# jianfenglihg/Unsupervised_depth_OpticalFlow_egomotion

Hardware: AMD Instinct MI355X
Metric: frame-pairs/sec (832x256, geom mode) (higher is better)
Workload: dtype f32; 1 GPU; train_step: mode=geom, 832x256, batch=4/GPU, num_scales=3, fwd+bwd+Adam; global_batch=4, parallelism=dp1, hw_queues=4, stream_priorities=auto

## Files before the change

### include/dfe_hip.h

```cpp
#ifndef DFE_HIP_H
#define DFE_HIP_H

#ifdef __cplusplus
extern "C" {
#endif

#define DFE_OK 0
#define DFE_ERR_NULL (-1)
#define DFE_ERR_DIMS (-2)
#define DFE_ERR_LAUNCH (-3)
#define DFE_ERR_UNSUPPORTED (-4)
#define DFE_ERR_WORKSPACE (-5)

#define DFE_MAX_SCALES 8
#define DFE_ABI_VERSION 4

int dfe_abi_version(void);
const char* dfe_error_string(int code);

int dfe_camera_floats(void);
int dfe_prepare_cameras(const float* pose, const float* K, float* cams, int B, int ndir, int nscale,
                        const float* downscale_host, void* stream);

int dfe_pose_vec2mat_fwd(const float* vec, float* T34, float* E, int n, void* stream);
// ... 121 lines not shown
int dfe_planeconv_dgrad(const float* gy, const float* weight, float* gx, float* ws, int B, int Ci, int Co, int H, int W,
                        void* stream);
int dfe_planeconv_wgrad(const float* gy, const float* x, float* gweight, float* ws, int B, int Ci, int Co, int H, int W,
                        void* stream);

long dfe_wino_weight_floats(int Ci, int Co);
long dfe_wino_scratch_floats(int B, int Ci, int Co, int H, int W, int P);
int dfe_wino_conv3x3(const float* x, const float* weight, float* y, long y_batch_stride, float* wbuf, long wbuf_floats, int B, int Ci,
                     int Co, int H, int W, int P, int transposed_weight, void* stream);
long dfe_wino_wgrad_floats(int B, int Ci, int Co, int H, int W, int P);
int dfe_wino_wgrad_tune(int tile, int blocks1, int blocks2, int chunk);
int dfe_wino_wgrad3x3(const float* x, long x_batch_stride, const float* gy, long gy_batch_stride, float* gweight, float* ws, int B,
                      int Ci, int Co, int H, int W, int P, void* stream);
int dfe_sconv_tune(int blocks, int rows);
long dfe_sconv_wgrad_floats(int B, int Ci, int Co, int H, int W, int K, int stride, int P);
int dfe_sconv_wgrad(const float* x, long x_batch_stride, const float* gy, long gy_batch_stride, float* gweight, float* ws, int B,
                    int Ci, int Co, int H, int W, int K, int stride, int P, void* stream);
long dfe_sconv_fwd_floats(int B, int Ci, int Co, int H, int W, int K);
int dfe_sconv_fwd(const float* x, long x_batch_stride, const float* weight, const float* bias, float slope, float* y,
                  long y_batch_stride, float* ws, int B, int Ci, int Co, int H, int W, int K, void* stream);
long dfe_sconv_dgrad_floats(int B, int Ci, int Co, int H, int W, int K);
int dfe_sconv_dgrad(const float* gy, long gy_batch_stride, const float* weight, float* gx, long gx_batch_stride, float* ws, int B,
                    int Ci, int Co, int H, int W, int K, void* stream);
int dfe_conv1x1s2_supported(int B, int Ci, int Co, int H, int W);
int dfe_conv1x1s2_fwd(const float* x, long x_batch_stride, const float* weight, float* y, long y_batch_stride, int B, int Ci, int Co,
                      int H, int W, void* stream);
long dfe_conv1x1s2_wgrad_floats(int B, int Ci, int Co, int H, int W);
int dfe_conv1x1s2_wgrad(const float* x, long x_batch_stride, const float* gy, long gy_batch_stride, float* gweight, float* ws, int B,
                        int Ci, int Co, int H, int W, void* stream);
int dfe_wino_conv3x3_dilated(const float* x, const float* weight, float* y, long y_batch_stride, float* wbuf, int B, int Ci, int Co,
                             int H, int W, int dilation, int transposed_weight, void* stream);
long dfe_wino_transform_blocks(int Ci, int Co);
int dfe_wino_transform_weights_multi(const long* table, const int* blockmap, int n_blocks, void* stream);
int dfe_wino_conv3x3_u(const float* x, const float* U, float* y, long y_batch_stride, float* part, long part_floats, int B, int Ci,
                       int Co, int H, int W, int P, int dilation, void* stream);
int dfe_wino_conv3x3_u_act(const float* x, const float* U, const float* bias, float slope, float* y, long y_batch_stride, float* y2,
                           long y2_batch_stride, float* part, long part_floats, int B, int Ci, int Co, int H, int W, int P,
                           int dilation, void* stream);

int dfe_conv1x1_small_supported(int B, int Ci, int Co, int H, int W);
int dfe_conv1x1_small_fwd(const float* x, const float* weight, const float* bias, float slope, float* y, int B, int Ci, int Co,
                          int H, int W, void* stream);
int dfe_conv1x1_small_bwd(const float* gy, const float* x, const float* weight, float* gx, float* gweight, int B, int Ci, int Co,
                          int H, int W, void* stream);

long dfe_bn_partials_floats(int G, int Bg, int C, int H, int W);
int dfe_bn_fwd(const float* x, const float* residual, const float* weight, const float* bias, float* running_mean,
               float* running_var, float* y, float* save_mean, float* save_invstd, float* partials, int G, int Bg, int C,
               int H, int W, float eps, float momentum, int relu, void* stream);
int dfe_bn_bwd(const float* x, const float* y, const float* gy, const float* weight, const float* save_mean,
               const float* save_invstd, float* gx, float* gres, float* gweight, float* gbias, float* partials,
               float* scratch_means, int G, int Bg, int C, int H, int W, int relu, void* stream);

int dfe_bn_fold(const float* weight, const float* bias, const float* running_mean, const float* running_var, float eps,
                float* scale, float* shift, int C, void* stream);
int dfe_bn_eval_fwd(const float* x, const float* residual, const float* scale, const float* shift, float* y, int B, int C, int H,
                    int W, int relu, void* stream);

long dfe_bias_act_partials_floats(int B, int C, int H, int W);
int dfe_bias_act_fwd(float* z, const float* bias, int B, int C, int H, int W, float slope, void* stream);
int dfe_bias_act_bwd(const float* y, const float* gy, long gy_batch_stride, float* gz, float* gbias, float* partials,
                     int B, int C, int H, int W, float slope, void* stream);

int dfe_bias_act_fwd2(const float* z, const float* bias, float* dst1, long dst1_batch_stride, float* dst2,
                      long dst2_batch_stride, int B, int C, int H, int W, float slope, void* stream);
int dfe_bias_act_bwd2(const float* y, long y_batch_stride, const float* g1, long g1_batch_stride, const float* g2,
                      long g2_batch_stride, float* gz, float* gbias, float* partials, int B, int C, int H, int W,
                      float slope, void* stream);
int dfe_bias_grad_final_multi(const float* const* partials, float* const* gbias, const int* C, int n, int B, int H, int W,
                              void* stream);

#define DFE_LOSS_DEPTH_PIXEL 0
#define DFE_LOSS_DEPTH_SMOOTH 1
#define DFE_LOSS_FLOW_PIXEL 2
#define DFE_LOSS_FLOW_SSIM 3
#define DFE_LOSS_FLOW_SMOOTH 4
#define DFE_LOSS_FLOW_CONSIS 5
#define DFE_LOSS_DEPTH_FLOW_CONSIS 6
#define DFE_LOSS_EPIPOLAR 7
#define DFE_LOSS_DEPTH_SSIM 8
#define DFE_LOSS_DEPTH_CONSIS 9
#define DFE_NUM_LOSSES 10
#define DFE_DEPTH_TERM_SSIM 1
#define DFE_DEPTH_TERM_CONSIS 2

#define DFE_MASK_VALID_BWD 0x01
#define DFE_MASK_VALID_FWD 0x02
#define DFE_MASK_OCC_BWD 0x04
#define DFE_MASK_OCC_FWD 0x08
#define DFE_MASK_DYNA_BWD 0x10
#define DFE_MASK_DYNA_FWD 0x20
#define DFE_MASK_TEX_BWD 0x40
#define DFE_MASK_TEX_FWD 0x80

typedef struct dfe_geom_args {
  int B, H, W;
  int num_scales;
  int align_corners;
  int mode;
  float alpha, beta;
  const float* img[3];
  const float* disp[3][DFE_MAX_SCALES];
  const float* flow[2][DFE_MAX_SCALES];
  const float* pose;
  const float* K;
  const float* K_inv;
// ... 33 lines not shown
```

### unsupervised_depth_opticalflow_egomotion_amd/csrc/dfe_internal.h

```cpp
#pragma once
#include <hip/hip_runtime.h>
#include <cstdint>
#include <cstdlib>
#include "../../include/dfe_hip.h"

#define DFE_LAUNCH_CHECK() do { if (hipGetLastError() != hipSuccess) return DFE_ERR_LAUNCH; } while (0)

namespace dfe {
struct ScaleList { float v[DFE_MAX_SCALES]; };
struct IntList { int v[DFE_MAX_SCALES]; };

inline int launch_status() { return hipGetLastError() == hipSuccess ? DFE_OK : DFE_ERR_LAUNCH; }
inline int env_int(const char* name, int dflt) { const char* e = getenv(name); return e ? atoi(e) : dflt; }
inline bool aligned8(const void* p) { return (reinterpret_cast<uintptr_t>(p) & 7) == 0; }
inline bool aligned16(const void* p) { return (reinterpret_cast<uintptr_t>(p) & 15) == 0; }
inline bool sample_ok(long bs, long per) { return bs >= per && per < (1L << 30); }
template <auto Kern, class... Args>
inline void launch_dyn_lds(unsigned grid, size_t lds_bytes, int attr_bytes, hipStream_t st, Args... args) {
  static bool attr_set = false;
  if (!attr_set) { (void)hipFuncSetAttribute(reinterpret_cast<const void*>(Kern), hipFuncAttributeMaxDynamicSharedMemorySize, attr_bytes); attr_set = true; }
  Kern<<<grid, 256, lds_bytes, st>>>(args...);
}

int launch_corr_fwd(const float* f1, const float* f2, float* out, long obs, float* tail, const float* flow, int B, int C, int H, int W,
                    hipStream_t st);
int launch_corr_bwd(const float* f1, const float* f2, const float* gout, long gbs, const float* add1, long abs1, float* g1,
                    float* g2, unsigned* amax2, int B, int C, int H, int W, hipStream_t st);

int launch_bias_final(const float* part, float* gbias, int B, int C, int n, hipStream_t st);
}
```

### unsupervised_depth_opticalflow_egomotion_amd/csrc/ops_bn.hip

```cpp
#include "dfe_internal.h"
#include "dfe_device.h"
#include "dfe_chunk.h"
#include <hip/hip_runtime.h>

namespace dfe {

constexpr int BN_BLOCK = CHUNK_BLOCK;
constexpr int BN_PER_THREAD = CHUNK_PER_THREAD;
constexpr int BN_CHUNK = CHUNK_ELEMS;

__device__ __forceinline__ float block_allsum(float v, float* smem) {
  v = dpp_add<0xB1>(v); v = dpp_add<0x4E>(v); v = dpp_add<0x141>(v); v = dpp_add<0x140>(v);
  const int lane = threadIdx.x & 63, wave = threadIdx.x >> 6;
  if ((lane & 15) == 0) smem[wave * 4 + (lane >> 4)] = v;
  __syncthreads();
  float s = 0.0f;
#pragma unroll
  for (int k = 0; k < 4 * (BN_BLOCK / 64); ++k) s += smem[k];
  __syncthreads();
  return s;
}

template <bool VEC>
__global__ void __launch_bounds__(BN_BLOCK) k_bn_stats(const float* __restrict__ x, float* __restrict__ part, int HW) {
// ... 364 lines not shown
    if (VEC) {
#pragma unroll
      for (int k = 0; k < BNE_PER_LANE / 4; ++k) {
        const int e = base + (k * 64 + lane) * 4;
        float4 q = make_float4(0.f, 0.f, 0.f, 0.f), p = q;
        if (e < HW) {
          q = *reinterpret_cast<const float4*>(x + off + e);
          if (RES) p = *reinterpret_cast<const float4*>(res + off + e);
        }
        v[4 * k] = q.x; v[4 * k + 1] = q.y; v[4 * k + 2] = q.z; v[4 * k + 3] = q.w;
        r[4 * k] = p.x; r[4 * k + 1] = p.y; r[4 * k + 2] = p.z; r[4 * k + 3] = p.w;
      }
    } else {
#pragma unroll
      for (int k = 0; k < BNE_PER_LANE; ++k) {
        const int e = base + k * 64 + lane;
        v[k] = e < HW ? x[off + e] : 0.0f;
        r[k] = (RES && e < HW) ? res[off + e] : 0.0f;
      }
    }
#pragma unroll
    for (int k = 0; k < BNE_PER_LANE; ++k) {
      float o = v[k] * s;
      o = o + t;
      if (RES) o = o + r[k];
      v[k] = (relu && o <= 0.0f) ? 0.0f : o;
    }
    if (VEC) {
#pragma unroll
      for (int k = 0; k < BNE_PER_LANE / 4; ++k) {
        const int e = base + (k * 64 + lane) * 4;
        if (e < HW) *reinterpret_cast<float4*>(y + off + e) = make_float4(v[4 * k], v[4 * k + 1], v[4 * k + 2], v[4 * k + 3]);
      }
    } else {
#pragma unroll
      for (int k = 0; k < BNE_PER_LANE; ++k) {
        const int e = base + k * 64 + lane;
        if (e < HW) y[off + e] = v[k];
      }
    }
  }
}

}

using namespace dfe;

static inline int bn_nchunk(long hw) { return static_cast<int>((hw + BN_CHUNK - 1) / BN_CHUNK); }

static int bn_dims(int G, int Bg, int C, int H, int W) {
  const long hw = static_cast<long>(H) * W;
  if (G <= 0 || Bg <= 0 || C <= 0 || H <= 0 || W <= 0 || hw >= (1L << 31) || C > 65535 || static_cast<long>(G) * Bg > 65535) return DFE_ERR_DIMS;
  if (static_cast<long>(Bg) * hw < 2) return DFE_ERR_DIMS;
  return DFE_OK;
}

extern "C" long dfe_bn_partials_floats(int G, int Bg, int C, int H, int W) {
  if (bn_dims(G, Bg, C, H, W) != DFE_OK) return 0;
  return static_cast<long>(G) * Bg * C * bn_nchunk(static_cast<long>(H) * W) * 3;
}

extern "C" int dfe_bn_fwd(const float* x, const float* residual, const float* weight, const float* bias, float* running_mean,
                          float* running_var, float* y, float* save_mean, float* save_invstd, float* partials, int G, int Bg,
                          int C, int H, int W, float eps, float momentum, int relu, void* stream) {
  if (!x || !y || !save_mean || !save_invstd || !partials) return DFE_ERR_NULL;
  int rc = bn_dims(G, Bg, C, H, W);
  if (rc != DFE_OK) return rc;
  const int hw = H * W, nchunk = bn_nchunk(hw);
  const dim3 grid(nchunk, C, G * Bg);
  hipStream_t st = static_cast<hipStream_t>(stream);
  const bool vec = hw % 4 == 0 && aligned16(x) && aligned16(y) && (!residual || aligned16(residual));
  if (vec && hw <= BNS_MAXHW && Bg <= BNS_MAXB) {
#define DFE_BNS_FWD(GB, T) k_bn_fwd_small<GB, T><<<C, T, 0, st>>>(x, residual, weight, bias, running_mean, running_var, y, \
                                                                save_mean, save_invstd, G, Bg, C, hw, eps, momentum, relu)
    if (G == 3) { if (hw <= 256) DFE_BNS_FWD(3, 64); else if (hw <= 1024) DFE_BNS_FWD(3, 256); else DFE_BNS_FWD(3, 1024); }
    else { if (hw <= 256) DFE_BNS_FWD(1, 64); else if (hw <= 1024) DFE_BNS_FWD(1, 256); else DFE_BNS_FWD(1, 1024); }
#undef DFE_BNS_FWD
    DFE_LAUNCH_CHECK();
    return DFE_OK;
  }
  if (vec) k_bn_stats<true><<<grid, BN_BLOCK, 0, st>>>(x, partials, hw);
  else k_bn_stats<false><<<grid, BN_BLOCK, 0, st>>>(x, partials, hw);
  DFE_LAUNCH_CHECK();
  k_bn_finalize<<<C, 64, 0, st>>>(partials, save_mean, save_invstd, running_mean, running_var, G, Bg, C, nchunk, eps, momentum);
  DFE_LAUNCH_CHECK();
  if (vec) k_bn_apply<true><<<grid, BN_BLOCK, 0, st>>>(x, residual, weight, bias, save_mean, save_invstd, y, Bg, C, hw, relu);
  else k_bn_apply<false><<<grid, BN_BLOCK, 0, st>>>(x, residual, weight, bias, save_mean, save_invstd, y, Bg, C, hw, relu);
  DFE_LAUNCH_CHECK();
  return DFE_OK;
}

extern "C" int dfe_bn_bwd(const float* x, const float* y, const float* gy, const float* weight, const float* save_mean,
                          const float* save_invstd, float* gx, float* gres, float* gweight, float* gbias, float* partials,
                          float* scratch_means, int G, int Bg, int C, int H, int W, int relu, void* stream) {
  if (!x || !gy || !save_mean || !save_invstd || !gx || !partials || !scratch_means || (relu && !y)) return DFE_ERR_NULL;
  int rc = bn_dims(G, Bg, C, H, W);
  if (rc != DFE_OK) return rc;
  const int hw = H * W, nchunk = bn_nchunk(hw);
  const dim3 grid(nchunk, C, G * Bg);
  hipStream_t st = static_cast<hipStream_t>(stream);
  float* gmean = scratch_means;
  float* gxmean = scratch_means + static_cast<long>(G) * C;
  const bool vec = hw % 4 == 0 && aligned16(x) && aligned16(gy) && aligned16(gx) && (!relu || aligned16(y)) && (!gres || aligned16(gres));
  if (vec && hw <= BNS_MAXHW && Bg <= BNS_MAXB) {
#define DFE_BNS_BWD(GB, T) k_bn_bwd_small<GB, T><<<C, T, 0, st>>>(x, y, gy, weight, save_mean, save_invstd, gx, gres, gweight, \
                                                                gbias, G, Bg, C, hw, relu)
    if (G == 3) { if (hw <= 256) DFE_BNS_BWD(3, 64); else if (hw <= 1024) DFE_BNS_BWD(3, 256); else DFE_BNS_BWD(3, 1024); }
    else { if (hw <= 256) DFE_BNS_BWD(1, 64); else if (hw <= 1024) DFE_BNS_BWD(1, 256); else DFE_BNS_BWD(1, 1024); }
#undef DFE_BNS_BWD
    DFE_LAUNCH_CHECK();
    return DFE_OK;
  }
  if (vec) k_bn_bwd_reduce<true><<<grid, BN_BLOCK, 0, st>>>(x, y, gy, save_mean, save_invstd, partials, Bg, C, hw, relu);
  else k_bn_bwd_reduce<false><<<grid, BN_BLOCK, 0, st>>>(x, y, gy, save_mean, save_invstd, partials, Bg, C, hw, relu);
  DFE_LAUNCH_CHECK();
  k_bn_bwd_finalize<<<C, 64, 0, st>>>(partials, gmean, gxmean, gweight, gbias, G, Bg, C, nchunk, hw);
  DFE_LAUNCH_CHECK();
  if (vec) k_bn_bwd_apply<true><<<grid, BN_BLOCK, 0, st>>>(x, y, gy, weight, save_mean, save_invstd, gmean, gxmean, gx, gres, Bg, C, hw, relu);
  else k_bn_bwd_apply<false><<<grid, BN_BLOCK, 0, st>>>(x, y, gy, weight, save_mean, save_invstd, gmean, gxmean, gx, gres, Bg, C, hw, relu);
  DFE_LAUNCH_CHECK();
  return DFE_OK;
}

extern "C" int dfe_bn_fold(const float* weight, const float* bias, const float* running_mean, const float* running_var, float eps,
                           float* scale, float* shift, int C, void* stream) {
  if (!running_mean || !running_var || !scale || !shift) return DFE_ERR_NULL;
  if (C <= 0) return DFE_ERR_DIMS;
  k_bn_fold<<<(C + 63) / 64, 64, 0, static_cast<hipStream_t>(stream)>>>(weight, bias, running_mean, running_var, eps, scale, shift, C);
  DFE_LAUNCH_CHECK();
  return DFE_OK;
}

extern "C" int dfe_bn_eval_fwd(const float* x, const float* residual, const float* scale, const float* shift, float* y, int B, int C,
                               int H, int W, int relu, void* stream) {
  if (!x || !scale || !shift || !y) return DFE_ERR_NULL;
  const long hw = static_cast<long>(H) * W;
  if (B <= 0 || C <= 0 || H <= 0 || W <= 0 || hw >= (1L << 31)) return DFE_ERR_DIMS;
  const long nchunk = (hw + BNE_WAVE_ELEMS - 1) / BNE_WAVE_ELEMS, units = static_cast<long>(B) * C * nchunk;
  if (units >= (1L << 30)) return DFE_ERR_DIMS;
  const long blocks = (units + BNE_WAVES - 1) / BNE_WAVES;
  const int grid = static_cast<int>(blocks < BNE_MAX_BLOCKS ? blocks : BNE_MAX_BLOCKS);
  hipStream_t st = static_cast<hipStream_t>(stream);
  const bool vec = hw % 4 == 0 && aligned16(x) && aligned16(y) && (!residual || aligned16(residual));
#define DFE_BNE(VEC, RES) k_bn_eval<VEC, RES><<<grid, BNE_BLOCK, 0, st>>>(x, residual, scale, shift, y, C, static_cast<int>(hw), \
                                                                          static_cast<int>(nchunk), static_cast<int>(units), relu)
  if (vec) { if (residual) DFE_BNE(true, true); else DFE_BNE(true, false); }
  else { if (residual) DFE_BNE(false, true); else DFE_BNE(false, false); }
#undef DFE_BNE
  DFE_LAUNCH_CHECK();
  return DFE_OK;
}
```

### unsupervised_depth_opticalflow_egomotion_amd/csrc/ops_pool.hip

```cpp
#include "dfe_device.h"
#include "dfe_internal.h"
#include <cmath>

namespace dfe {

constexpr int PL_ROWS = 8;

struct Row3 { float v0, v1, v2; };

__device__ __forceinline__ Row3 pool_row(const float* __restrict__ plane, int r, int H, int W, int ox, bool lane_live) {
  const float ninf = -INFINITY;
  Row3 o{ninf, ninf, ninf};
  const bool rok = lane_live && r >= 0 && r < H;
  const int c1 = 2 * ox;
  if (rok) {
    const float* row = plane + static_cast<long>(r) * W;
    if (c1 + 1 < W) { const PairF p = *reinterpret_cast<const PairF*>(row + c1); o.v1 = p.a; o.v2 = p.b; }
    else o.v1 = row[c1];
  }
  const float left = wave_shr1(o.v2);
  o.v0 = left;
  if ((threadIdx.x & 63) == 0) o.v0 = (rok && c1 - 1 >= 0) ? plane[static_cast<long>(r) * W + c1 - 1] : ninf;
  if (ox == 0) o.v0 = ninf;
  return o;
}

__device__ __forceinline__ void pool_scan(const Row3& r, int base, float& best, int& bi, bool& seeded, int rr, int H, int ox, int W, int oy) {
  const int row = 2 * oy - 1 + rr;
  if (row < 0 || row >= H) return;
  const float v[3] = {r.v0, r.v1, r.v2};
#pragma unroll
  for (int cc = 0; cc < 3; ++cc) {
    const int col = 2 * ox - 1 + cc;
    if (col < 0 || col >= W) continue;
    if (!seeded) { bi = base + cc; seeded = true; }
    if (v[cc] > best || v[cc] != v[cc]) { best = v[cc]; bi = base + cc; }
  }
}

__global__ void __launch_bounds__(64) k_maxpool3x3s2_fwd(const float* __restrict__ x, float* __restrict__ y,
                                                         unsigned char* __restrict__ idx, int H, int W, int Ho, int Wo,
                                                         int strips) {
  const int strip = blockIdx.x % strips, rb = blockIdx.x / strips;
  const long pl = blockIdx.y;
  const int ox = strip * 64 + static_cast<int>(threadIdx.x);
  const bool live = ox < Wo;
  const float* plane = x + pl * H * W;
  const int oy0 = rb * PL_ROWS, oy1 = min(oy0 + PL_ROWS, Ho);
  Row3 top = pool_row(plane, 2 * oy0 - 1, H, W, ox, live);
  for (int oy = oy0; oy < oy1; ++oy) {
    const Row3 mid = pool_row(plane, 2 * oy, H, W, ox, live);
    const Row3 bot = pool_row(plane, 2 * oy + 1, H, W, ox, live);
    float best = -INFINITY;
    int bi = 0;
    bool seeded = false;
    pool_scan(top, 0, best, bi, seeded, 0, H, ox, W, oy);
    pool_scan(mid, 3, best, bi, seeded, 1, H, ox, W, oy);
    pool_scan(bot, 6, best, bi, seeded, 2, H, ox, W, oy);
    if (live) {
      const long o = (pl * Ho + oy) * Wo + ox;
      y[o] = best;
      idx[o] = static_cast<unsigned char>(bi);
    }
    top = bot;
  }
}

struct GI { float g; int k; };

__device__ __forceinline__ GI pool_gi(const float* __restrict__ gy, const unsigned char* __restrict__ idx, long plane_off,
                                      int oy, int ox, int Ho, int Wo) {
  GI r{0.0f, -1};
  if (oy >= 0 && oy < Ho && ox >= 0 && ox < Wo) {
    const long o = plane_off + static_cast<long>(oy) * Wo + ox;
    r.g = gy[o]; r.k = idx[o];
  }
  return r;
}

__global__ void __launch_bounds__(64) k_maxpool3x3s2_bwd(const float* __restrict__ gy, const unsigned char* __restrict__ idx,
                                                         float* __restrict__ gx, int H, int W, int Ho, int Wo, int strips) {
  const int strip = blockIdx.x % strips, rb = blockIdx.x / strips;
  const long pl = blockIdx.y;
  const int ox = strip * 64 + static_cast<int>(threadIdx.x);
  const int c1 = 2 * ox, c2 = 2 * ox + 1;
  if (c1 >= W) return;
  const long po = pl * Ho * Wo;
  float* plane = gx + pl * H * W;
  const int oy0 = rb * PL_ROWS, oy1 = min(oy0 + PL_ROWS, Ho);
  GI pa = pool_gi(gy, idx, po, oy0 - 1, ox, Ho, Wo), pb = pool_gi(gy, idx, po, oy0 - 1, ox + 1, Ho, Wo);
// ... 52 lines not shown
```

### unsupervised_depth_opticalflow_egomotion_amd/networks/depth_model.py

```python
import numpy as np
import torch
import torch.nn as nn
import torch.nn.functional as F

from . import resnet
from .. import convs, ops


class ResnetEncoder(nn.Module):
    def __init__(self, num_layers=18, pretrained=False):
        super().__init__()
        if num_layers not in (18, 34):
            raise ValueError("{} is not a valid number of resnet layers".format(num_layers))
        self.num_ch_enc = np.array([64, 64, 128, 256, 512])
        self.encoder = {18: resnet.resnet18, 34: resnet.resnet34}[num_layers](pretrained)

    def forward(self, image):
        e = self.encoder
        x = (image - 0.45) / 0.225
        f0 = e.bn1(e.conv1(x), relu=True)
        f1 = e.layer1(e.maxpool(f0))
        f2 = e.layer2(f1)
        f3 = e.layer3(f2)
        f4 = e.layer4(f3)
        return [f0, f1, f2, f3, f4]


class Conv3x3(nn.Module):

    def __init__(self, cin, cout):
        super().__init__()
        self.pad = nn.ReflectionPad2d(1)
        self.conv = nn.Conv2d(int(cin), int(cout), 3)

    def forward(self, x):
        return self.conv(self.pad(x))


class ConvBlock(nn.Module):

    def __init__(self, cin, cout):
        super().__init__()
        self.conv = Conv3x3(cin, cout)
        self.nonlin = nn.ELU(inplace=True)

    def forward(self, x):
        return self.nonlin(self.conv(x))


class DepthDecoder(nn.Module):
    def __init__(self, num_ch_enc, scales=range(4)):
        super().__init__()
        self.scales = list(scales)
        self.num_ch_enc = num_ch_enc
        self.num_ch_dec = np.array([16, 32, 64, 128, 256])
        self.upconvs = nn.ModuleList()
        for i in range(4, -1, -1):
            cin = num_ch_enc[-1] if i == 4 else self.num_ch_dec[i + 1]
            pair = nn.ModuleList([ConvBlock(cin, self.num_ch_dec[i])])
            cin2 = self.num_ch_dec[i] + (num_ch_enc[i - 1] if i > 0 else 0)
            pair.append(ConvBlock(cin2, self.num_ch_dec[i]))
            self.upconvs.append(pair)
        self.dispconvs = nn.ModuleList([Conv3x3(self.num_ch_dec[s], 1) for s in self.scales])
        self.sigmoid = nn.Sigmoid()

    def forward(self, feats):
        return self.forward_fused(feats) if feats[-1].is_cuda else self.forward_aten(feats)

    def forward_aten(self, feats):
        out = {}
        x = feats[-1]
        for scale in range(4, -1, -1):
            blk = self.upconvs[4 - scale]
            x = blk[0](x)
# ... 58 lines not shown
```

### unsupervised_depth_opticalflow_egomotion_amd/networks/resnet.py

```python
import torch
import torch.nn as nn
import torch.nn.functional as F

from .. import ops
from ..convs import Conv2d


class FrameBatchNorm2d(nn.BatchNorm2d):
    groups = 1
    count_deferred = False
    folded = None

    def forward(self, x, residual=None, relu=False):
        if self.folded is not None and x.is_cuda and not self.training:
            return ops.bn_eval(x, self.folded[0], self.folded[1], residual=residual, relu=relu, out=x if x.is_contiguous() else None)
        if x.is_cuda and self.training:
            if self.momentum is None or not self.track_running_stats or not self.affine:
                raise ValueError("FrameBatchNorm2d: only affine, momentum-tracked batch norm is implemented in HIP")
            if not self.count_deferred:
                self.num_batches_tracked.add_(self.groups)
            return ops.grouped_batch_norm(x, self.weight, self.bias, self.running_mean, self.running_var, self.groups,
                                          self.eps, self.momentum, residual=residual, relu=relu)
        if self.training and self.groups > 1:
            y = torch.cat([super(FrameBatchNorm2d, self).forward(c) for c in x.chunk(self.groups, 0)], 0)
        else:
            y = super().forward(x)
        if residual is not None:
            y = y + residual
        return F.relu(y) if relu else y


class StemMaxPool(nn.MaxPool2d):

    def forward(self, x):
        if x.is_cuda and (self.kernel_size, self.stride, self.padding, self.dilation, self.ceil_mode) == (3, 2, 1, 1, False) \
                and x.dim() == 4 and x.shape[0] * x.shape[1] <= 65535:
            return ops.maxpool3x3s2(x)
        return super().forward(x)


class BasicBlock(nn.Module):
    expansion = 1

    def __init__(self, inplanes, planes, stride=1, downsample=None):
        super().__init__()
        self.conv1 = Conv2d(inplanes, planes, 3, stride, 1, bias=False)
        self.bn1 = FrameBatchNorm2d(planes)
        self.relu = nn.ReLU(inplace=True)
        self.conv2 = Conv2d(planes, planes, 3, 1, 1, bias=False)
        self.bn2 = FrameBatchNorm2d(planes)
        self.downsample = downsample
        self.stride = stride

    def forward(self, x):
        idt = x if self.downsample is None else self.downsample(x)
        out = self.bn1(self.conv1(x), relu=True)
        return self.bn2(self.conv2(out), residual=idt, relu=True)


class ResNet(nn.Module):
    def __init__(self, block, layers, num_classes=1000):
        super().__init__()
        self.inplanes = 64
        self.conv1 = Conv2d(3, 64, 7, 2, 3, bias=False)
        self.bn1 = FrameBatchNorm2d(64)
        self.relu = nn.ReLU(inplace=True)
        self.maxpool = StemMaxPool(3, 2, 1)
        self.layer1 = self._make_layer(block, 64, layers[0])
        self.layer2 = self._make_layer(block, 128, layers[1], stride=2)
        self.layer3 = self._make_layer(block, 256, layers[2], stride=2)
        self.layer4 = self._make_layer(block, 512, layers[3], stride=2)
        self.avgpool = nn.AdaptiveAvgPool2d((1, 1))
        self.fc = nn.Linear(512 * block.expansion, num_classes)
        for m in self.modules():
            if isinstance(m, nn.Conv2d):
                nn.init.kaiming_normal_(m.weight, mode="fan_out", nonlinearity="relu")
            elif isinstance(m, nn.BatchNorm2d):
                nn.init.constant_(m.weight, 1)
                nn.init.constant_(m.bias, 0)

    def _make_layer(self, block, planes, blocks, stride=1):
        down = None
        if stride != 1 or self.inplanes != planes * block.expansion:
            down = nn.Sequential(Conv2d(self.inplanes, planes * block.expansion, 1, stride, bias=False),
                                 FrameBatchNorm2d(planes * block.expansion))
        layers = [block(self.inplanes, planes, stride, down)]
        self.inplanes = planes * block.expansion
        layers += [block(self.inplanes, planes) for _ in range(1, blocks)]
        return nn.Sequential(*layers)

    def forward(self, x):
        x = self.maxpool(self.bn1(self.conv1(x), relu=True))
        x = self.layer4(self.layer3(self.layer2(self.layer1(x))))
        return self.fc(self.avgpool(x).flatten(1))


def resnet18(pretrained=False, **kw):
    if pretrained:
        raise RuntimeError("no network access: pretrained ImageNet weights are unavailable")
    return ResNet(BasicBlock, [2, 2, 2, 2], **kw)


def resnet34(pretrained=False, **kw):
    if pretrained:
        raise RuntimeError("no network access: pretrained ImageNet weights are unavailable")
    return ResNet(BasicBlock, [3, 4, 6, 3], **kw)
```

### unsupervised_depth_opticalflow_egomotion_amd/ops.py

```python
from __future__ import annotations

import ctypes
import os
import threading

import torch

from . import _lib
from ._lib import DfeError, check, f32c, get_lib, ptr, stream_ptr

_ALIGN_CORNERS = False


def set_align_corners(flag: bool):
    global _ALIGN_CORNERS
    _ALIGN_CORNERS = bool(flag)


def get_align_corners() -> bool:
    return _ALIGN_CORNERS


def _ac(flag):
    return int(_ALIGN_CORNERS if flag is None else bool(flag))
# ... 1031 lines not shown
    @staticmethod
    def forward(ctx, x, residual, weight, bias, running_mean, running_var, groups, eps, momentum, relu):
        lib = get_lib()
        x = f32c(x)
        N, C, H, W = x.shape
        G = int(groups)
        if N % G:
            raise ValueError("batch %d is not divisible into %d groups" % (N, G))
        Bg = N // G
        residual = f32c(residual) if residual is not None else None
        if residual is not None and residual.shape != x.shape:
            raise ValueError("residual must have the shape of x")
        dev = x.device
        y = torch.empty_like(x)
        mean = torch.empty(G * C, device=dev)
        invstd = torch.empty(G * C, device=dev)
        npart = lib.dfe_bn_partials_floats(G, Bg, C, H, W)
        part = torch.empty(max(npart, 1), device=dev)
        check(lib.dfe_bn_fwd(ptr(x), ptr(residual), ptr(weight), ptr(bias), ptr(running_mean), ptr(running_var), ptr(y),
                             ptr(mean), ptr(invstd), ptr(part), G, Bg, C, H, W, float(eps), float(momentum), int(relu),
                             stream_ptr()), "dfe_bn_fwd")
        ctx.save_for_backward(x, y if relu else x.new_empty(0), weight if weight is not None else x.new_empty(0), mean, invstd)
        ctx.cfg = (G, Bg, C, H, W, int(relu), residual is not None, weight is not None)
        ctx.mark_non_differentiable(mean, invstd)
        return y

    @staticmethod
    def backward(ctx, gy):
        lib = get_lib()
        x, y, weight, mean, invstd = ctx.saved_tensors
        G, Bg, C, H, W, relu, has_res, has_w = ctx.cfg
        gy = f32c(gy)
        dev = x.device
        gx = torch.empty_like(x)
        gres = (torch.empty_like(x) if relu else None) if (has_res and ctx.needs_input_grad[1]) else None
        gw = torch.empty(C, device=dev) if (has_w and ctx.needs_input_grad[2]) else None
        gb = torch.empty(C, device=dev) if ctx.needs_input_grad[3] else None
        part = torch.empty(max(lib.dfe_bn_partials_floats(G, Bg, C, H, W), 1), device=dev)
        scratch = torch.empty(2 * G * C, device=dev)
        check(lib.dfe_bn_bwd(ptr(x), ptr(y) if relu else None, ptr(gy), ptr(weight) if has_w else None, ptr(mean), ptr(invstd),
                             ptr(gx), ptr(gres), ptr(gw), ptr(gb), ptr(part), ptr(scratch), G, Bg, C, H, W, relu,
                             stream_ptr()), "dfe_bn_bwd")
        if has_res and ctx.needs_input_grad[1] and not relu:
            gres = gy
        return gx, gres, gw, gb, None, None, None, None, None, None


def grouped_batch_norm(x, weight, bias, running_mean, running_var, groups=1, eps=1e-5, momentum=0.1, residual=None,
                       relu=False):
    return GroupedBatchNormFn.apply(x, residual, weight, bias, running_mean, running_var, int(groups), float(eps),
                                    float(momentum), bool(relu))


def _forward_only(what, *tensors):
    if torch.is_grad_enabled() and any(t is not None and t.requires_grad for t in tensors):
        raise DfeError("%s is forward-only (it has no backward pass): call it under torch.no_grad(), or detach its inputs" % what)


def bn_fold(bn, out=None):
    if bn.running_mean is None or bn.running_var is None:
        raise DfeError("bn_fold: the layer tracks no running statistics")
    _forward_only("bn_fold", bn.weight, bn.bias, bn.running_mean, bn.running_var)
    C = int(bn.running_mean.numel())
    scale, shift = out if out is not None else (torch.empty(C, device=bn.running_mean.device, dtype=torch.float32) for _ in range(2))
    for t in (scale, shift):
        if t.dtype != torch.float32 or t.numel() != C:
            raise DfeError("bn_fold: out must be two fp32 tensors of %d elements" % C)
    w, b = (None if t is None else f32c(t.detach()) for t in (bn.weight, bn.bias))
    check(get_lib().dfe_bn_fold(ptr(w), ptr(b), ptr(f32c(bn.running_mean)), ptr(f32c(bn.running_var)), float(bn.eps), ptr(scale),
                                ptr(shift), C, stream_ptr()), "dfe_bn_fold")
    return scale, shift


def bn_eval(x, scale, shift, residual=None, relu=False, out=None):
    _forward_only("bn_eval", x, scale, shift, residual)
    if x.dim() != 4:
        raise DfeError("bn_eval: x must be [B,C,H,W], got %s" % (tuple(x.shape),))
    x = x if out is x else f32c(x)
    B, C, H, W = x.shape
    residual = f32c(residual) if residual is not None else None
    if residual is not None and residual.shape != x.shape:
        raise DfeError("bn_eval: residual must have the shape of x")
    if any(t.dtype != torch.float32 or t.numel() != C for t in (scale, shift)):
        raise DfeError("bn_eval: scale / shift must be fp32 tensors of %d channels (ops.bn_fold's)" % C)
    y = torch.empty_like(x) if out is None else out
    if y.shape != x.shape or y.dtype != torch.float32 or x.dtype != torch.float32:
        raise DfeError("bn_eval: out must be an fp32 tensor of the shape of x")
    if residual is not None and residual.data_ptr() == y.data_ptr():
        raise DfeError("bn_eval: residual must not alias out")
    check(get_lib().dfe_bn_eval_fwd(ptr(x), ptr(residual), ptr(scale), ptr(shift), ptr(y), B, C, H, W, int(bool(relu)), stream_ptr()),
          "dfe_bn_eval_fwd")
    return y


class DispHeadFn(torch.autograd.Function):

    @staticmethod
    def forward(ctx, p, weight, bias):
        lib = get_lib()
        p, weight = f32c(p), f32c(weight)
        bias = f32c(bias) if bias is not None else None
        B, C, Hp, Wp = p.shape
        if tuple(weight.shape) != (1, C, 3, 3):
            raise ValueError("weight must be [1,%d,3,3], got %s" % (C, tuple(weight.shape)))
        H, W = Hp - 2, Wp - 2
        out = torch.empty(B, 1, H, W, device=p.device)
# ... 70 lines not shown
```

Baseline: 434.3 frame-pairs/s.

## Fuse ResNet stem BatchNorm apply, ReLU and 3x3 max-pool into one kernel pair

Adds a fused stem op that computes BN statistics, then applies the BN affine and ReLU while producing the stride-2 3x3 max-pool output and argmax positions in a single pass. The backward routes pooled gradients back through the stored argmax and the ReLU mask inside the BN backward reduce and apply kernels, so no separate maxpool backward or intermediate gradient tensor is needed. This cuts kernel launches and full-resolution memory traffic for the stem. In exchange it adds more complex index logic, extra uint8 position storage, and recomputes the pool-gradient scatter in both the reduce and the apply kernel.

```diff
diff --git a/include/dfe_hip.h b/include/dfe_hip.h
--- a/include/dfe_hip.h
+++ b/include/dfe_hip.h
@@ -197,6 +197,13 @@
                const float* save_invstd, float* gx, float* gres, float* gweight, float* gbias, float* partials,
                float* scratch_means, int G, int Bg, int C, int H, int W, int relu, void* stream);
 
+int dfe_bn_relu_pool_fwd(const float* x, const float* weight, const float* bias, float* running_mean, float* running_var,
+                         float* f0, float* pooled, unsigned char* pos, float* save_mean, float* save_invstd, float* partials,
+                         int G, int Bg, int C, int H, int W, float eps, float momentum, void* stream);
+int dfe_bn_relu_pool_bwd(const float* x, const float* weight, const float* bias, const float* save_mean, const float* save_invstd,
+                         const float* g_f0, const float* g_pooled, const unsigned char* pos, float* gx, float* gweight,
+                         float* gbias, float* partials, float* scratch_means, int G, int Bg, int C, int H, int W, void* stream);
+
 int dfe_bn_fold(const float* weight, const float* bias, const float* running_mean, const float* running_var, float eps,
                 float* scale, float* shift, int C, void* stream);
 int dfe_bn_eval_fwd(const float* x, const float* residual, const float* scale, const float* shift, float* y, int B, int C, int H,
diff --git a/unsupervised_depth_opticalflow_egomotion_amd/csrc/dfe_internal.h b/unsupervised_depth_opticalflow_egomotion_amd/csrc/dfe_internal.h
--- a/unsupervised_depth_opticalflow_egomotion_amd/csrc/dfe_internal.h
+++ b/unsupervised_depth_opticalflow_egomotion_amd/csrc/dfe_internal.h
@@ -27,5 +27,10 @@
 int launch_corr_bwd(const float* f1, const float* f2, const float* gout, long gbs, const float* add1, long abs1, float* g1,
                     float* g2, unsigned* amax2, int B, int C, int H, int W, hipStream_t st);
 
+int launch_bn_stats(const float* x, float* running_mean, float* running_var, float* save_mean, float* save_invstd, float* partials,
+                    int G, int Bg, int C, int H, int W, bool vec, float eps, float momentum, hipStream_t st);
+int launch_bn_bwd_finalize(const float* partials, float* gmean, float* gxmean, float* gweight, float* gbias, int G, int Bg, int C,
+                           int H, int W, hipStream_t st);
+
 int launch_bias_final(const float* part, float* gbias, int B, int C, int n, hipStream_t st);
 }
diff --git a/unsupervised_depth_opticalflow_egomotion_amd/csrc/dfe_pool.h b/unsupervised_depth_opticalflow_egomotion_amd/csrc/dfe_pool.h
--- /dev/null
+++ b/unsupervised_depth_opticalflow_egomotion_amd/csrc/dfe_pool.h
@@ -0,0 +1,23 @@
+#pragma once
+#include <hip/hip_runtime.h>
+
+namespace dfe {
+
+constexpr int PL_ROWS = 8;
+
+struct Row3 { float v0, v1, v2; };
+
+__device__ __forceinline__ void pool_scan(const Row3& r, int base, float& best, int& bi, bool& seeded, int rr, int H, int ox, int W, int oy) {
+  const int row = 2 * oy - 1 + rr;
+  if (row < 0 || row >= H) return;
+  const float v[3] = {r.v0, r.v1, r.v2};
+#pragma unroll
+  for (int cc = 0; cc < 3; ++cc) {
+    const int col = 2 * ox - 1 + cc;
+    if (col < 0 || col >= W) continue;
+    if (!seeded) { bi = base + cc; seeded = true; }
+    if (v[cc] > best || v[cc] != v[cc]) { best = v[cc]; bi = base + cc; }
+  }
+}
+
+}
diff --git a/unsupervised_depth_opticalflow_egomotion_amd/csrc/ops_bn.hip b/unsupervised_depth_opticalflow_egomotion_amd/csrc/ops_bn.hip
--- a/unsupervised_depth_opticalflow_egomotion_amd/csrc/ops_bn.hip
+++ b/unsupervised_depth_opticalflow_egomotion_amd/csrc/ops_bn.hip
@@ -440,6 +440,29 @@
   const long hw = static_cast<long>(H) * W;
   if (G <= 0 || Bg <= 0 || C <= 0 || H <= 0 || W <= 0 || hw >= (1L << 31) || C > 65535 || static_cast<long>(G) * Bg > 65535) return DFE_ERR_DIMS;
   if (static_cast<long>(Bg) * hw < 2) return DFE_ERR_DIMS;
+  return DFE_OK;
+}
+
+int dfe::launch_bn_stats(const float* x, float* running_mean, float* running_var, float* save_mean, float* save_invstd,
+                         float* partials, int G, int Bg, int C, int H, int W, bool vec, float eps, float momentum, hipStream_t st) {
+  const int rc = bn_dims(G, Bg, C, H, W);
+  if (rc != DFE_OK) return rc;
+  const int hw = H * W, nchunk = bn_nchunk(hw);
+  const dim3 grid(nchunk, C, G * Bg);
+  if (vec) k_bn_stats<true><<<grid, BN_BLOCK, 0, st>>>(x, partials, hw);
+  else k_bn_stats<false><<<grid, BN_BLOCK, 0, st>>>(x, partials, hw);
+  DFE_LAUNCH_CHECK();
+  k_bn_finalize<<<C, 64, 0, st>>>(partials, save_mean, save_invstd, running_mean, running_var, G, Bg, C, nchunk, eps, momentum);
+  DFE_LAUNCH_CHECK();
+  return DFE_OK;
+}
+
+int dfe::launch_bn_bwd_finalize(const float* partials, float* gmean, float* gxmean, float* gweight, float* gbias, int G, int Bg,
+                                int C, int H, int W, hipStream_t st) {
+  const int rc = bn_dims(G, Bg, C, H, W);
+  if (rc != DFE_OK) return rc;
+  k_bn_bwd_finalize<<<C, 64, 0, st>>>(partials, gmean, gxmean, gweight, gbias, G, Bg, C, bn_nchunk(static_cast<long>(H) * W), H * W);
+  DFE_LAUNCH_CHECK();
   return DFE_OK;
 }
 
@@ -467,11 +490,8 @@
     DFE_LAUNCH_CHECK();
     return DFE_OK;
   }
-  if (vec) k_bn_stats<true><<<grid, BN_BLOCK, 0, st>>>(x, partials, hw);
-  else k_bn_stats<false><<<grid, BN_BLOCK, 0, st>>>(x, partials, hw);
-  DFE_LAUNCH_CHECK();
-  k_bn_finalize<<<C, 64, 0, st>>>(partials, save_mean, save_invstd, running_mean, running_var, G, Bg, C, nchunk, eps, momentum);
-  DFE_LAUNCH_CHECK();
+  rc = launch_bn_stats(x, running_mean, running_var, save_mean, save_invstd, partials, G, Bg, C, H, W, vec, eps, momentum, st);
+  if (rc != DFE_OK) return rc;
   if (vec) k_bn_apply<true><<<grid, BN_BLOCK, 0, st>>>(x, residual, weight, bias, save_mean, save_invstd, y, Bg, C, hw, relu);
   else k_bn_apply<false><<<grid, BN_BLOCK, 0, st>>>(x, residual, weight, bias, save_mean, save_invstd, y, Bg, C, hw, relu);
   DFE_LAUNCH_CHECK();
@@ -502,8 +522,8 @@
   if (vec) k_bn_bwd_reduce<true><<<grid, BN_BLOCK, 0, st>>>(x, y, gy, save_mean, save_invstd, partials, Bg, C, hw, relu);
   else k_bn_bwd_reduce<false><<<grid, BN_BLOCK, 0, st>>>(x, y, gy, save_mean, save_invstd, partials, Bg, C, hw, relu);
   DFE_LAUNCH_CHECK();
-  k_bn_bwd_finalize<<<C, 64, 0, st>>>(partials, gmean, gxmean, gweight, gbias, G, Bg, C, nchunk, hw);
-  DFE_LAUNCH_CHECK();
+  rc = launch_bn_bwd_finalize(partials, gmean, gxmean, gweight, gbias, G, Bg, C, H, W, st);
+  if (rc != DFE_OK) return rc;
   if (vec) k_bn_bwd_apply<true><<<grid, BN_BLOCK, 0, st>>>(x, y, gy, weight, save_mean, save_invstd, gmean, gxmean, gx, gres, Bg, C, hw, relu);
   else k_bn_bwd_apply<false><<<grid, BN_BLOCK, 0, st>>>(x, y, gy, weight, save_mean, save_invstd, gmean, gxmean, gx, gres, Bg, C, hw, relu);
   DFE_LAUNCH_CHECK();
diff --git a/unsupervised_depth_opticalflow_egomotion_amd/csrc/ops_pool.hip b/unsupervised_depth_opticalflow_egomotion_amd/csrc/ops_pool.hip
--- a/unsupervised_depth_opticalflow_egomotion_amd/csrc/ops_pool.hip
+++ b/unsupervised_depth_opticalflow_egomotion_amd/csrc/ops_pool.hip
@@ -1,12 +1,9 @@
 #include "dfe_device.h"
 #include "dfe_internal.h"
+#include "dfe_pool.h"
 #include <cmath>
 
 namespace dfe {
-
-constexpr int PL_ROWS = 8;
-
-struct Row3 { float v0, v1, v2; };
 
 __device__ __forceinline__ Row3 pool_row(const float* __restrict__ plane, int r, int H, int W, int ox, bool lane_live) {
   const float ninf = -INFINITY;
@@ -23,19 +20,6 @@
   if ((threadIdx.x & 63) == 0) o.v0 = (rok && c1 - 1 >= 0) ? plane[static_cast<long>(r) * W + c1 - 1] : ninf;
   if (ox == 0) o.v0 = ninf;
   return o;
-}
-
-__device__ __forceinline__ void pool_scan(const Row3& r, int base, float& best, int& bi, bool& seeded, int rr, int H, int ox, int W, int oy) {
-  const int row = 2 * oy - 1 + rr;
-  if (row < 0 || row >= H) return;
-  const float v[3] = {r.v0, r.v1, r.v2};
-#pragma unroll
-  for (int cc = 0; cc < 3; ++cc) {
-    const int col = 2 * ox - 1 + cc;
-    if (col < 0 || col >= W) continue;
-    if (!seeded) { bi = base + cc; seeded = true; }
-    if (v[cc] > best || v[cc] != v[cc]) { best = v[cc]; bi = base + cc; }
-  }
 }
 
 __global__ void __launch_bounds__(64) k_maxpool3x3s2_fwd(const float* __restrict__ x, float* __restrict__ y,
diff --git a/unsupervised_depth_opticalflow_egomotion_amd/csrc/ops_stem.hip b/unsupervised_depth_opticalflow_egomotion_amd/csrc/ops_stem.hip
--- /dev/null
+++ b/unsupervised_depth_opticalflow_egomotion_amd/csrc/ops_stem.hip
@@ -0,0 +1,253 @@
+#include "dfe_device.h"
+#include "dfe_internal.h"
+#include "dfe_chunk.h"
+#include "dfe_pool.h"
+#include <cmath>
+
+namespace dfe {
+
+struct StemAffine { float mu, is, sc, sh; };
+
+__device__ __forceinline__ StemAffine stem_affine(const float* __restrict__ weight, const float* __restrict__ bias,
+                                                  const float* __restrict__ mean, const float* __restrict__ invstd, int plane,
+                                                  int Bg, int C) {
+  const int n = plane / C, c = plane - n * C, g = n / Bg;
+  const float is = invstd[g * C + c];
+  return StemAffine{mean[g * C + c], is, is * (weight ? weight[c] : 1.0f), bias ? bias[c] : 0.0f};
+}
+
+__device__ __forceinline__ float stem_pre(float v, const StemAffine& a) { return (v - a.mu) * a.sc + a.sh; }
+__device__ __forceinline__ float stem_act(float v, const StemAffine& a) {
+  const float o = stem_pre(v, a);
+  return o <= 0.0f ? 0.0f : o;
+}
+
+constexpr int ST_IN_ROWS = 2 * PL_ROWS + 1;
+
+__global__ void __launch_bounds__(64) k_stem_apply_pool(const float* __restrict__ x, const float* __restrict__ weight,
+                                                        const float* __restrict__ bias, const float* __restrict__ mean,
+                                                        const float* __restrict__ invstd, float* __restrict__ f0,
+                                                        float* __restrict__ y, unsigned char* __restrict__ idx, int Bg, int C,
+                                                        int H, int W, int Ho, int Wo, int strips) {
+  const int strip = blockIdx.x % strips, rb = blockIdx.x / strips;
+  const long pl = blockIdx.y;
+  const StemAffine a = stem_affine(weight, bias, mean, invstd, static_cast<int>(blockIdx.y), Bg, C);
+  const int ox = strip * 64 + static_cast<int>(threadIdx.x);
+  const bool live = ox < Wo;
+  const int c1 = 2 * ox;
+  const bool pair = c1 + 1 < W;
+  const bool first = threadIdx.x == 0;
+  const float* xp = x + pl * H * W;
+  float* fp = f0 + pl * H * W;
+  const int oy0 = rb * PL_ROWS, oy1 = min(oy0 + PL_ROWS, Ho);
+  const int r0 = 2 * oy0 - 1;
+  float xa[ST_IN_ROWS], xb[ST_IN_ROWS], xl[ST_IN_ROWS];
+#pragma unroll
+  for (int t = 0; t < ST_IN_ROWS; ++t) {
+    const int r = r0 + t;
+    xa[t] = 0.0f; xb[t] = 0.0f; xl[t] = 0.0f;
+    if (live && r >= 0 && r < H) {
+      const float* row = xp + static_cast<long>(r) * W;
+      if (pair) { const PairF p = *reinterpret_cast<const PairF*>(row + c1); xa[t] = p.a; xb[t] = p.b; }
+      else xa[t] = row[c1];
+      if (first && ox > 0) xl[t] = row[c1 - 1];
+    }
+  }
+  const float ninf = -INFINITY;
+  auto make_row = [&](int t) -> Row3 {
+    const int r = r0 + t;
+    const bool rok = live && r >= 0 && r < H;
+    Row3 o{ninf, ninf, ninf};
+    if (rok) {
+      o.v1 = stem_act(xa[t], a);
+      if (pair) o.v2 = stem_act(xb[t], a);
+      if (t > 0) {
+        float* row = fp + static_cast<long>(r) * W;
+        if (pair) *reinterpret_cast<PairF*>(row + c1) = PairF{o.v1, o.v2}; else row[c1] = o.v1;
+      }
+    }
+    o.v0 = wave_shr1(o.v2);
+    if (first) o.v0 = (rok && ox > 0) ? stem_act(xl[t], a) : ninf;
+    if (ox == 0) o.v0 = ninf;
+    return o;
+  };
+  Row3 top = make_row(0);
+#pragma unroll
+  for (int i = 0; i < PL_ROWS; ++i) {
+    const int oy = oy0 + i;
+    if (oy >= oy1) break;
+    const Row3 mid = make_row(2 * i + 1);
+    const Row3 bot = make_row(2 * i + 2);
+    float best = ninf;
+    int bi = 0;
+    bool seeded = false;
+    pool_scan(top, 0, best, bi, seeded, 0, H, ox, W, oy);
+    pool_scan(mid, 3, best, bi, seeded, 1, H, ox, W, oy);
+    pool_scan(bot, 6, best, bi, seeded, 2, H, ox, W, oy);
+    if (live) {
+      const long o = (pl * Ho + oy) * Wo + ox;
+      y[o] = best;
+      idx[o] = static_cast<unsigned char>(bi);
+    }
+    top = bot;
+  }
+}
+
+struct PoolGrad { const float* g; const unsigned char* k; int W, Ho, Wo; };
+
+__device__ __forceinline__ void stem_adj_row1(const PoolGrad& p, int oy, int wr, int c, float& s) {
+  if (oy >= p.Ho) return;
+  const long o = static_cast<long>(oy) * p.Wo + (c >> 1);
+  const int b = 3 * wr;
+  const int k0 = p.k[o];
+  const float g0 = p.g[o];
+  if ((c & 1) == 0) { if (k0 == b + 1) s += g0; return; }
+  const bool second = (c >> 1) + 1 < p.Wo;
+  const int k1 = second ? p.k[o + 1] : -1;
+  const float g1 = second ? p.g[o + 1] : 0.0f;
+  if (k0 == b + 2) s += g0;
+  if (k1 == b) s += g1;
+}
+
+__device__ __forceinline__ void stem_adj_row4(const PoolGrad& p, int oy, int wr, int c0, float (&s)[4]) {
+  if (oy >= p.Ho) return;
+  const long o = static_cast<long>(oy) * p.Wo + (c0 >> 1);
+  const int b = 3 * wr;
+  const bool third = (c0 >> 1) + 2 < p.Wo;
+  const int k0 = p.k[o], k1 = p.k[o + 1], k2 = third ? p.k[o + 2] : -1;
+  const float g0 = p.g[o], g1 = p.g[o + 1], g2 = third ? p.g[o + 2] : 0.0f;
+  if (k0 == b + 1) s[0] += g0;
+  if (k0 == b + 2) s[1] += g0;
+  if (k1 == b) s[1] += g1;
+  if (k1 == b + 1) s[2] += g1;
+  if (k1 == b + 2) s[3] += g1;
+  if (k2 == b) s[3] += g2;
+}
+
+template <bool VEC>
+__device__ __forceinline__ void stem_grad8(const float* __restrict__ xp, const float* __restrict__ gsp, const PoolGrad& p,
+                                           const StemAffine& a, int base, int HW, float (&v)[CHUNK_PER_THREAD],
+                                           float (&gm)[CHUNK_PER_THREAD]) {
+  bool ok[CHUNK_PER_THREAD];
+  float gs[CHUNK_PER_THREAD], adj[CHUNK_PER_THREAD];
+  load8<VEC>(xp, base, HW, v, ok);
+  if (gsp) load8<VEC>(gsp, base, HW, gs, ok);
+#pragma unroll
+  for (int k = 0; k < CHUNK_PER_THREAD; ++k) adj[k] = 0.0f;
+  if (p.g) {
+    if (VEC && p.W % 4 == 0) {
+#pragma unroll
+      for (int q = 0; q < CHUNK_PER_THREAD / 4; ++q) {
+        const int e = base + (q * CHUNK_BLOCK + static_cast<int>(threadIdx.x)) * 4;
+        if (e >= HW) continue;
+        const int r = e / p.W, c0 = e - r * p.W;
+        float s[4] = {0.0f, 0.0f, 0.0f, 0.0f};
+        if (r & 1) { stem_adj_row4(p, (r - 1) >> 1, 2, c0, s); stem_adj_row4(p, (r + 1) >> 1, 0, c0, s); }
+        else stem_adj_row4(p, r >> 1, 1, c0, s);
+#pragma unroll
+        for (int j = 0; j < 4; ++j) adj[4 * q + j] = s[j];
+      }
+    } else {
+#pragma unroll
+      for (int k = 0; k < CHUNK_PER_THREAD; ++k) {
+        const int e = VEC ? base + ((k >> 2) * CHUNK_BLOCK + static_cast<int>(threadIdx.x)) * 4 + (k & 3)
+                          : base + k * CHUNK_BLOCK + static_cast<int>(threadIdx.x);
+        if (e >= HW) continue;
+        const int r = e / p.W, c = e - r * p.W;
+        float s = 0.0f;
+        if (r & 1) { stem_adj_row1(p, (r - 1) >> 1, 2, c, s); stem_adj_row1(p, (r + 1) >> 1, 0, c, s); }
+        else stem_adj_row1(p, r >> 1, 1, c, s);
+        adj[k] = s;
+      }
+    }
+  }
+#pragma unroll
+  for (int k = 0; k < CHUNK_PER_THREAD; ++k) {
+    const float g = p.g ? (gsp ? gs[k] + adj[k] : adj[k]) : gs[k];
+    gm[k] = (!ok[k] || stem_pre(v[k], a) <= 0.0f) ? 0.0f : g;
+  }
+}
+
+#define DFE_STEM_BWD_PARAMS const float* __restrict__ x, const float* __restrict__ g_f0, const float* __restrict__ g_pooled, \
+    const unsigned char* __restrict__ pos, const float* __restrict__ weight, const float* __restrict__ bias,                 \
+    const float* __restrict__ mean, const float* __restrict__ invstd
+
+template <bool VEC>
+__global__ void __launch_bounds__(CHUNK_BLOCK) k_stem_bwd_reduce(DFE_STEM_BWD_PARAMS, float* __restrict__ part, int Bg, int C,
+                                                                 int H, int W, int Ho, int Wo) {
+  __shared__ float red[2 * 4 * (CHUNK_BLOCK / 64)];
+  const long pl = plane_id();
+  const StemAffine a = stem_affine(weight, bias, mean, invstd, static_cast<int>(pl), Bg, C);
+  const PoolGrad p{g_pooled ? g_pooled + pl * Ho * Wo : nullptr, pos + pl * Ho * Wo, W, Ho, Wo};
+  const int HW = H * W, base = blockIdx.x * CHUNK_ELEMS;
+  float v[CHUNK_PER_THREAD], gm[CHUNK_PER_THREAD];
+  stem_grad8<VEC>(x + pl * HW, g_f0 ? g_f0 + pl * HW : nullptr, p, a, base, HW, v, gm);
+  float acc[2] = {0.0f, 0.0f};
+#pragma unroll
+  for (int k = 0; k < CHUNK_PER_THREAD; ++k) {
+    acc[0] += gm[k];
+    acc[1] += gm[k] * ((v[k] - a.mu) * a.is);
+  }
+  block_sum<2>(acc, red, part + (pl * gridDim.x + blockIdx.x) * 2);
+}
+
+template <bool VEC>
+__global__ void __launch_bounds__(CHUNK_BLOCK) k_stem_bwd_apply(DFE_STEM_BWD_PARAMS, const float* __restrict__ gmean,
+                                                                const float* __restrict__ gxmean, float* __restrict__ gx, int Bg,
+                                                                int C, int H, int W, int Ho, int Wo) {
+  const long pl = plane_id();
+  const StemAffine a = stem_affine(weight, bias, mean, invstd, static_cast<int>(pl), Bg, C);
+  const int n = static_cast<int>(pl) / C, c = static_cast<int>(pl) - n * C, g = n / Bg;
+  const float ws = (weight ? weight[c] : 1.0f) * a.is, m0 = gmean[g * C + c], m1 = gxmean[g * C + c];
+  const PoolGrad p{g_pooled ? g_pooled + pl * Ho * Wo : nullptr, pos + pl * Ho * Wo, W, Ho, Wo};
+  const int HW = H * W, base = blockIdx.x * CHUNK_ELEMS;
+  float v[CHUNK_PER_THREAD], gm[CHUNK_PER_THREAD];
+  stem_grad8<VEC>(x + pl * HW, g_f0 ? g_f0 + pl * HW : nullptr, p, a, base, HW, v, gm);
+#pragma unroll
+  for (int k = 0; k < CHUNK_PER_THREAD; ++k) v[k] = ws * ((gm[k] - m0) - ((v[k] - a.mu) * a.is) * m1);
+  store8<VEC>(gx + pl * HW, base, HW, v);
+}
+#undef DFE_STEM_BWD_PARAMS
+
+}
+
+using namespace dfe;
+
+extern "C" int dfe_bn_relu_pool_fwd(const float* x, const float* weight, const float* bias, float* running_mean, float* running_var,
+                                    float* f0, float* pooled, unsigned char* pos, float* save_mean, float* save_invstd,
+                                    float* partials, int G, int Bg, int C, int H, int W, float eps, float momentum, void* stream) {
+  if (!x || !f0 || !pooled || !pos || !save_mean || !save_invstd || !partials) return DFE_ERR_NULL;
+  if (G <= 0 || Bg <= 0 || C <= 0 || static_cast<long>(G) * Bg * C > 65535) return DFE_ERR_DIMS;
+  hipStream_t st = static_cast<hipStream_t>(stream);
+  const bool vec = (static_cast<long>(H) * W) % 4 == 0 && aligned16(x) && aligned16(f0);
+  const int rc = launch_bn_stats(x, running_mean, running_var, save_mean, save_invstd, partials, G, Bg, C, H, W, vec, eps, momentum, st);
+  if (rc != DFE_OK) return rc;
+  const int Ho = dfe_maxpool3x3s2_out(H), Wo = dfe_maxpool3x3s2_out(W);
+  const int strips = (Wo + 63) / 64, rbs = (Ho + PL_ROWS - 1) / PL_ROWS;
+  k_stem_apply_pool<<<dim3(strips * rbs, G * Bg * C), 64, 0, st>>>(x, weight, bias, save_mean, save_invstd, f0, pooled, pos, Bg, C,
+                                                                  H, W, Ho, Wo, strips);
+  return launch_status();
+}
+
+extern "C" int dfe_bn_relu_pool_bwd(const float* x, const float* weight, const float* bias, const float* save_mean,
+                                    const float* save_invstd, const float* g_f0, const float* g_pooled, const unsigned char* pos,
+                                    float* gx, float* gweight, float* gbias, float* partials, float* scratch_means, int G, int Bg,
+                                    int C, int H, int W, void* stream) {
+  if (!x || !save_mean || !save_invstd || !pos || !gx || !partials || !scratch_means || (!g_f0 && !g_pooled)) return DFE_ERR_NULL;
+  if (dfe_bn_partials_floats(G, Bg, C, H, W) == 0) return DFE_ERR_DIMS;
+  hipStream_t st = static_cast<hipStream_t>(stream);
+  const int hw = H * W, nchunk = (hw + CHUNK_ELEMS - 1) / CHUNK_ELEMS;
+  const int Ho = dfe_maxpool3x3s2_out(H), Wo = dfe_maxpool3x3s2_out(W);
+  const dim3 grid(nchunk, C, G * Bg);
+  float* gmean = scratch_means;
+  float* gxmean = scratch_means + static_cast<long>(G) * C;
+  const bool vec = hw % 4 == 0 && aligned16(x) && aligned16(gx) && (!g_f0 || aligned16(g_f0));
+  if (vec) k_stem_bwd_reduce<true><<<grid, CHUNK_BLOCK, 0, st>>>(x, g_f0, g_pooled, pos, weight, bias, save_mean, save_invstd, partials, Bg, C, H, W, Ho, Wo);
+  else k_stem_bwd_reduce<false><<<grid, CHUNK_BLOCK, 0, st>>>(x, g_f0, g_pooled, pos, weight, bias, save_mean, save_invstd, partials, Bg, C, H, W, Ho, Wo);
+  DFE_LAUNCH_CHECK();
+  const int rc = launch_bn_bwd_finalize(partials, gmean, gxmean, gweight, gbias, G, Bg, C, H, W, st);
+  if (rc != DFE_OK) return rc;
+  if (vec) k_stem_bwd_apply<true><<<grid, CHUNK_BLOCK, 0, st>>>(x, g_f0, g_pooled, pos, weight, bias, save_mean, save_invstd, gmean, gxmean, gx, Bg, C, H, W, Ho, Wo);
+  else k_stem_bwd_apply<false><<<grid, CHUNK_BLOCK, 0, st>>>(x, g_f0, g_pooled, pos, weight, bias, save_mean, save_invstd, gmean, gxmean, gx, Bg, C, H, W, Ho, Wo);
+  return launch_status();
+}
diff --git a/unsupervised_depth_opticalflow_egomotion_amd/networks/depth_model.py b/unsupervised_depth_opticalflow_egomotion_amd/networks/depth_model.py
--- a/unsupervised_depth_opticalflow_egomotion_amd/networks/depth_model.py
+++ b/unsupervised_depth_opticalflow_egomotion_amd/networks/depth_model.py
@@ -18,8 +18,8 @@
     def forward(self, image):
         e = self.encoder
         x = (image - 0.45) / 0.225
-        f0 = e.bn1(e.conv1(x), relu=True)
-        f1 = e.layer1(e.maxpool(f0))
+        f0, pooled = resnet.stem_bn_relu_pool(e.bn1, e.maxpool, e.conv1(x))
+        f1 = e.layer1(pooled)
         f2 = e.layer2(f1)
         f3 = e.layer3(f2)
         f4 = e.layer4(f3)
diff --git a/unsupervised_depth_opticalflow_egomotion_amd/networks/resnet.py b/unsupervised_depth_opticalflow_egomotion_amd/networks/resnet.py
--- a/unsupervised_depth_opticalflow_egomotion_amd/networks/resnet.py
+++ b/unsupervised_depth_opticalflow_egomotion_amd/networks/resnet.py
@@ -32,11 +32,24 @@
 
 class StemMaxPool(nn.MaxPool2d):
 
+    def eligible(self, x):
+        return x.is_cuda and (self.kernel_size, self.stride, self.padding, self.dilation, self.ceil_mode) == (3, 2, 1, 1, False) \
+            and x.dim() == 4 and x.shape[0] * x.shape[1] <= 65535
+
     def forward(self, x):
-        if x.is_cuda and (self.kernel_size, self.stride, self.padding, self.dilation, self.ceil_mode) == (3, 2, 1, 1, False) \
-                and x.dim() == 4 and x.shape[0] * x.shape[1] <= 65535:
+        if self.eligible(x):
             return ops.maxpool3x3s2(x)
         return super().forward(x)
+
+
+def stem_bn_relu_pool(bn, pool, x):
+    if (x.is_cuda and bn.training and bn.folded is None and pool.eligible(x) and bn.affine and bn.track_running_stats
+            and bn.momentum is not None and ops.stem_fusable(x, bn.groups)):
+        if not bn.count_deferred:
+            bn.num_batches_tracked.add_(bn.groups)
+        return ops.bn_relu_pool(x, bn.weight, bn.bias, bn.running_mean, bn.running_var, bn.groups, bn.eps, bn.momentum)
+    f0 = bn(x, relu=True)
+    return f0, pool(f0)
 
 
 class BasicBlock(nn.Module):
@@ -90,7 +103,7 @@
         return nn.Sequential(*layers)
 
     def forward(self, x):
-        x = self.maxpool(self.bn1(self.conv1(x), relu=True))
+        x = stem_bn_relu_pool(self.bn1, self.maxpool, self.conv1(x))[1]
         x = self.layer4(self.layer3(self.layer2(self.layer1(x))))
         return self.fc(self.avgpool(x).flatten(1))
 
diff --git a/unsupervised_depth_opticalflow_egomotion_amd/ops.py b/unsupervised_depth_opticalflow_egomotion_amd/ops.py
--- a/unsupervised_depth_opticalflow_egomotion_amd/ops.py
+++ b/unsupervised_depth_opticalflow_egomotion_amd/ops.py
@@ -1107,6 +1107,75 @@
                                     float(momentum), bool(relu))
 
 
+STEM_FUSED = os.environ.get("DFE_STEM_FUSED", "1") != "0"
+
+
+def _bn_three_kernel(Bg, H, W):
+    hw = H * W
+    return not (hw % 4 == 0 and hw <= 4096 and Bg <= 4)
+
+
+def stem_fusable(x, groups):
+    return (STEM_FUSED and x.dim() == 4 and x.shape[0] % int(groups) == 0 and x.shape[0] * x.shape[1] <= 65535
+            and _bn_three_kernel(x.shape[0] // int(groups), x.shape[2], x.shape[3]))
+
+
+class BnReluPoolFn(torch.autograd.Function):
+
+    @staticmethod
+    def forward(ctx, x, weight, bias, running_mean, running_var, groups, eps, momentum):
+        lib = get_lib()
+        x = f32c(x)
+        N, C, H, W = x.shape
+        G = int(groups)
+        if N % G:
+            raise ValueError("batch %d is not divisible into %d groups" % (N, G))
+        Bg = N // G
+        dev = x.device
+        Ho, Wo = lib.dfe_maxpool3x3s2_out(H), lib.dfe_maxpool3x3s2_out(W)
+        f0 = torch.empty_like(x)
+        pooled = torch.empty(N, C, Ho, Wo, device=dev, dtype=torch.float32)
+        pos = torch.empty(N, C, Ho, Wo, device=dev, dtype=torch.uint8)
+        mean = torch.empty(G * C, device=dev)
+        invstd = torch.empty(G * C, device=dev)
+        part = torch.empty(max(lib.dfe_bn_partials_floats(G, Bg, C, H, W), 1), device=dev)
+        check(lib.dfe_bn_relu_pool_fwd(ptr(x), ptr(weight), ptr(bias), ptr(running_mean), ptr(running_var), ptr(f0), ptr(pooled),
+                                       ptr(pos), ptr(mean), ptr(invstd), ptr(part), G, Bg, C, H, W, float(eps), float(momentum),
+                                       stream_ptr()), "dfe_bn_relu_pool_fwd")
+        ctx.save_for_backward(x, weight, bias, mean, invstd, pos)
+        ctx.cfg = (G, Bg, C, H, W)
+        ctx.set_materialize_grads(False)
+        return f0, pooled
+
+    @staticmethod
+    def backward(ctx, g_f0, g_pooled):
+        if g_f0 is None and g_pooled is None:
+            return (None,) * 8
+        lib = get_lib()
+        x, weight, bias, mean, invstd, pos = ctx.saved_tensors
+        G, Bg, C, H, W = ctx.cfg
+        dev = x.device
+        g_f0 = f32c(g_f0) if g_f0 is not None else None
+        g_pooled = f32c(g_pooled) if g_pooled is not None else None
+        gx = torch.empty_like(x)
+        gw = torch.empty(C, device=dev) if (weight is not None and ctx.needs_input_grad[1]) else None
+        gb = torch.empty(C, device=dev) if (bias is not None and ctx.needs_input_grad[2]) else None
+        part = torch.empty(max(lib.dfe_bn_partials_floats(G, Bg, C, H, W), 1), device=dev)
+        scratch = torch.empty(2 * G * C, device=dev)
+        check(lib.dfe_bn_relu_pool_bwd(ptr(x), ptr(weight), ptr(bias), ptr(mean), ptr(invstd), ptr(g_f0), ptr(g_pooled), ptr(pos),
+                                       ptr(gx), ptr(gw), ptr(gb), ptr(part), ptr(scratch), G, Bg, C, H, W, stream_ptr()),
+              "dfe_bn_relu_pool_bwd")
+        return gx, gw, gb, None, None, None, None, None
+
+
+def bn_relu_pool(x, weight, bias, running_mean, running_var, groups=1, eps=1e-5, momentum=0.1):
+    if x.dim() != 4:
+        raise ValueError("bn_relu_pool: x must be [B,C,H,W]")
+    if x.shape[0] * x.shape[1] > 65535:
+        raise _lib.DfeError("bn_relu_pool: more than 65535 planes")
+    return BnReluPoolFn.apply(x, weight, bias, running_mean, running_var, int(groups), float(eps), float(momentum))
+
+
 def _forward_only(what, *tensors):
     if torch.is_grad_enabled() and any(t is not None and t.requires_grad for t in tensors):
         raise DfeError("%s is forward-only (it has no backward pass): call it under torch.no_grad(), or detach its inputs" % what)
```

Result: no change. 437.5 frame-pairs/s, median of 5 (+0.8%).
